# peteroh23/ModulationDetectionCNN

Measured on AMD Instinct MI355X. Metric: I/Q frames/sec (2x128, VT-CNN2, batch=2^20), higher is better.
Workload: dtype bf16; 1 GPU; vtcnn2-c11-bf16-n2^20; topology=vtcnn2, classes=11, frames_per_gpu=1048576, global_batch=1048576, parallelism=batch-shard x1 (no collective), outputs=softmax probabilities f32 + argmax int32, frames_per_forward_call=1048576, full=False

## Files before the change

modulationdetectioncnn_amd/csrc/vtcnn2_bf16_sched.hip:

```cpp
#include "vtcnn2_bf16_common.h"
#include "vtcnn2_sched_common.h"

#include <cmath>
#include <cstdlib>
#include <type_traits>

namespace mdc {

namespace {

constexpr int kNV = 24;

struct SchedState {
    u32x4 Wv[kNV];
    u32x4 Wa[kWFrags - kNV];
    f32x4 bias[5];
    u32x4 A1[2];
    unsigned Bf[2][2][2][4];
    f32x16 X[2];
    f32x4 rp[4];
    float rc[4];
    float tprev;
    u32x4 L0[3];
    u32x4 L1;
    unsigned cb[4];
    unsigned wr_addr, rd_addr, rc_addr, im_addr;
    int gs;
};

template <int SP, int J, int I, bool PAD = false>
__device__ __forceinline__ void sch_tap(SchedState& st, f32x4 (&acc)[5]) {
    constexpr int CT = 1 - I / 10, BB = (I / 5) % 2, OT = I % 5;
    constexpr int IDX = ((CT * 3 + J) * 2 + BB) * 5 + OT;
    const u32x4 b = u32x4{st.Bf[SP][CT][BB][0], st.Bf[SP][CT][BB][1], st.Bf[SP][CT][BB][2], st.Bf[SP][CT][BB][3]};
    if constexpr (J == 0 && I < 5) {
        if constexpr (IDX < kNV) asm volatile("v_mfma_f32_16x16x32_bf16 %0, %1, %2, %3" : "=&a"(acc[OT]) : "v"(st.Wv[IDX]), "v"(b), "a"(st.bias[OT]));
        else asm volatile("v_mfma_f32_16x16x32_bf16 %0, %1, %2, %3" : "=&a"(acc[OT]) : "a"(st.Wa[IDX - kNV]), "v"(b), "a"(st.bias[OT]));
    } else if constexpr (PAD) {
        static_assert(IDX >= kNV, "padded form written for the AGPR-resident fragments only");
        asm volatile("s_nop 1\n\tv_mfma_f32_16x16x32_bf16 %0, %1, %2, %0" : "+a"(acc[OT]) : "a"(st.Wa[IDX - kNV]), "v"(b));
    } else {
        if constexpr (IDX < kNV) asm volatile("v_mfma_f32_16x16x32_bf16 %0, %1, %2, %0" : "+a"(acc[OT]) : "v"(st.Wv[IDX]), "v"(b));
        else asm volatile("v_mfma_f32_16x16x32_bf16 %0, %1, %2, %0" : "+a"(acc[OT]) : "a"(st.Wa[IDX - kNV]), "v"(b));
    }
}
template <int SP, int U>
__device__ __forceinline__ void sch_packop(SchedState& st) {
    constexpr int CT = U >> 3, j = U & 7;
    unsigned& d = st.Bf[SP][CT][j >> 2][j & 3];
    const float lo = st.X[CT][2 * j], hi = st.X[CT][2 * j + 1];
    asm volatile("v_cvt_pk_bf16_f32 %0, %1, %2 clamp" : "=v"(d) : "v"(lo), "v"(hi));
}
template <int V12, bool FIRST, bool LAST, int ABL, bool RANGE = false>
__device__ __forceinline__ void sch_step(SchedState& st, int v, int q, unsigned short* fbase, f32x4 (&acc)[3][5], int wlo = 0) {
    constexpr int PAR = V12 & 1, PN = 1 - PAR;
    constexpr int R1 = (V12 + 1) & 3, S0 = ((V12 + 1) >> 2) % 3, SN = (S0 + 1) % 3;
    constexpr bool kLoadEven = (V12 & 3) == 1 && !LAST, kLoadOdd = (V12 & 3) == 3 && !LAST;
    constexpr int LSLOT = ((V12 >> 2) + 1) % 3;
    constexpr bool kExch = ABL != 2 && ABL != 6, kFin = ABL != 3 && ABL != 6, kC1 = ABL != 5 && ABL != 6;
    f32x4 (&a2)[5] = acc[V12 % 3];
    f32x4 (&a1)[5] = acc[(V12 + 1) % 3];
    f32x4 (&a0)[5] = acc[(V12 + 2) % 3];
    const unsigned load_addr = st.im_addr + ((v >> 2) * 16 + (kLoadEven ? 16 : 24));
    FinTmp ft;
    FinOut fo;
    constexpr int OP = (V12 + 1) & 1;
#define FIN(K) do { if (!FIRST && kFin) sch_fin_clamp<K, OP>(st, ft, fo); } while (0)
#define PREP(I) do { if (!LAST && kC1 && ABL != 11) sch_prep<R1, S0, SN, I>(st); } while (0)
#define C1M(CT) do { if (!LAST && kC1) sch_conv1_mfma<R1, S0, CT>(st); } while (0)
#define ST(W) do { if (!FIRST && kFin && (W == 0 || OP == 1)) { if (ABL == 7) { if (W == 0) asm volatile("" ::"v"(fo.o0), "v"(fo.o1)); else asm volatile("" ::"v"(fo.tt)); } else if (!RANGE || v - 1 >= wlo) sch_store<W>(fo, fbase, v - 1, q, st.gs); } } while (0)
#define WR(OT) do { if (kExch && ABL != 8) sch_part_write<PAR, OT>(st, a2[OT]); } while (0)
#define PK(N) do { if (!LAST && kC1 && ABL != 10) sch_packop<PN, N>(st); } while (0)
#define RD(R) do { if (kExch && ABL != 9) sch_red_load1<PAR, R>(st); } while (0)
#define LD() do { if (kC1 && ABL != 11) { if (kLoadEven) sch_load_even<LSLOT>(st, load_addr); else if (kLoadOdd) sch_load_odd(st, load_addr); } } while (0)
#ifdef MDC_F8_PROBE_HALF_BARRIER
    constexpr bool kHalfBarrierSkip = (V12 & 1) == 1;
#else
    constexpr bool kHalfBarrierSkip = false;
#endif
#define HANDOFF() do { \
        if (ABL == 1 || kHalfBarrierSkip) asm volatile("s_waitcnt lgkmcnt(0)" ::: "memory"); \
        else if (kExch) asm volatile("s_waitcnt lgkmcnt(0)\n\ts_barrier" ::: "memory"); \
        asm volatile("" ::"a"(a2[0]), "a"(a2[1]), "a"(a2[2]), "a"(a2[3]), "a"(a2[4])); } while (0)
    sch_wait_lds(st);
    sch_tap<PAR, 2, 0, RANGE && (V12 == 1 || V12 == 2)>(st, a2); FIN(0);
    sch_tap<PAR, 2, 1>(st, a2); FIN(1);
    sch_tap<PAR, 2, 2>(st, a2); FIN(2);
    sch_tap<PAR, 2, 3>(st, a2); FIN(3);
    sch_tap<PAR, 2, 4>(st, a2); FIN(4);
    sch_tap<PAR, 2, 5>(st, a2); FIN(5);
    sch_tap<PAR, 2, 6>(st, a2); FIN(6);
    sch_tap<PAR, 2, 7>(st, a2); FIN(7);
    sch_tap<PAR, 2, 8>(st, a2); FIN(8);
    sch_tap<PAR, 2, 9>(st, a2); FIN(9);
    sch_tap<PAR, 2, 10>(st, a2); FIN(10);
    sch_tap<PAR, 2, 11>(st, a2); FIN(11);
    sch_tap<PAR, 2, 12>(st, a2); FIN(12);
    sch_tap<PAR, 2, 13>(st, a2); FIN(13);
    sch_tap<PAR, 2, 14>(st, a2); FIN(14);
    sch_tap<PAR, 2, 15>(st, a2); FIN(15);
    sch_tap<PAR, 2, 16>(st, a2); PREP(0);
    sch_tap<PAR, 2, 17>(st, a2); PREP(1);
    sch_tap<PAR, 2, 18>(st, a2); PREP(2);
    sch_tap<PAR, 2, 19>(st, a2); PREP(3);
    C1M(0); WR(0); FIN(16); FIN(17);
    C1M(1); WR(1);
    sch_tap<PAR, 1, 0>(st, a1); ST(0);
    sch_tap<PAR, 1, 1>(st, a1); WR(2);
    sch_tap<PAR, 1, 2>(st, a1); ST(1);
    sch_tap<PAR, 1, 3>(st, a1); PK(0);
    sch_tap<PAR, 1, 4>(st, a1); WR(3);
    sch_tap<PAR, 1, 5>(st, a1); PK(1);
    sch_tap<PAR, 1, 6>(st, a1); PK(2);
    sch_tap<PAR, 1, 7>(st, a1); WR(4);
    sch_tap<PAR, 1, 8>(st, a1); PK(3);
    sch_tap<PAR, 1, 9>(st, a1); PK(4);
    sch_tap<PAR, 1, 10>(st, a1); PK(5);
    sch_tap<PAR, 1, 11>(st, a1); PK(6);
    sch_tap<PAR, 1, 12>(st, a1); PK(7);
    sch_tap<PAR, 1, 13>(st, a1); PK(8);
    sch_tap<PAR, 1, 14>(st, a1); PK(9);
    sch_tap<PAR, 1, 15>(st, a1); PK(10);
    sch_tap<PAR, 1, 16>(st, a1); PK(11);
    sch_tap<PAR, 1, 17>(st, a1); PK(12);
    sch_tap<PAR, 1, 18>(st, a1); PK(13);
    sch_tap<PAR, 1, 19>(st, a1); PK(14);
    sch_tap<PAR, 0, 0>(st, a0); PK(15);
    sch_tap<PAR, 0, 1>(st, a0);
    sch_tap<PAR, 0, 2>(st, a0);
    sch_tap<PAR, 0, 3>(st, a0);
    sch_tap<PAR, 0, 4>(st, a0);
    sch_tap<PAR, 0, 5>(st, a0);
    sch_tap<PAR, 0, 6>(st, a0); HANDOFF();
    sch_tap<PAR, 0, 7>(st, a0); RD(0);
    sch_tap<PAR, 0, 8>(st, a0); RD(1);
    sch_tap<PAR, 0, 9>(st, a0); RD(2);
    sch_tap<PAR, 0, 10>(st, a0); RD(3);
    sch_tap<PAR, 0, 11>(st, a0); RD(4);
    sch_tap<PAR, 0, 12>(st, a0); RD(5);
    sch_tap<PAR, 0, 13>(st, a0); RD(6);
    sch_tap<PAR, 0, 14>(st, a0); RD(7);
    sch_tap<PAR, 0, 15>(st, a0); LD();
    sch_tap<PAR, 0, 16>(st, a0);
    sch_tap<PAR, 0, 17>(st, a0);
    sch_tap<PAR, 0, 18>(st, a0);
    sch_tap<PAR, 0, 19>(st, a0);
    if (ABL == 10 && !LAST) asm volatile("" ::"v"(st.X[0]), "v"(st.X[1]));
#undef FIN
#undef PREP
#undef C1M
#undef ST
#undef WR
#undef PK
#undef RD
#undef LD
#undef HANDOFF
}

template <int ABL, bool U8 = false, bool RANGE = false>
__global__ __launch_bounds__(256, 1) void vt_conv_bf16_sched_kernel(const float* __restrict__ x, long n,
                                                                    const u32x4* __restrict__ wq, const u32x4* __restrict__ a1q,
                                                                    const float* __restrict__ b2, unsigned short* __restrict__ feat,
                                                                    long hop2 = 256, float scale = 0.f) {
    extern __shared__ __attribute__((aligned(16))) unsigned char smem[];
    unsigned* img = reinterpret_cast<unsigned*>(smem);
    const int tid = threadIdx.x, lane = tid & 63;
    const int q = __builtin_amdgcn_readfirstlane(tid >> 6);
    const int nl = lane & 15, g = lane >> 4;

    SchedState st;
#pragma unroll
    for (int i = 0; i < kWFrags; ++i) {
        const u32x4 w = wq[(q * kWFrags + i) * 64 + lane];
        if (i < kNV) { st.Wv[i] = w; asm volatile("" : "+v"(st.Wv[i])); }
        else { st.Wa[i - kNV] = w; asm volatile("" : "+a"(st.Wa[i - kNV])); }
    }
    st.A1[0] = a1q[(q * 2 + 0) * 64 + lane];
    st.A1[1] = a1q[(q * 2 + 1) * 64 + lane];
#pragma unroll
    for (int ot = 0; ot < 5; ++ot) {
        const f32x4 b = *reinterpret_cast<const f32x4*>(b2 + 16 * ot + 4 * g);
        st.bias[ot] = q == 0 ? b : f32x4{0.f, 0.f, 0.f, 0.f};
        asm volatile("" : "+a"(st.bias[ot]));
    }
    const unsigned part_lds = (unsigned)(size_t)(__attribute__((address_space(3))) unsigned char*)(smem + (size_t)2 * kSImgWords * 4);
    const unsigned img_lds = (unsigned)(size_t)(__attribute__((address_space(3))) unsigned char*)smem;
    auto entry = [](int f, int gg) { return 8 * (4 * (f >> 3) + gg) + ((f & 7) ^ (gg >> 1)); };
    const int fs = lane >> 2, gs = lane & 3;
    st.gs = gs;
    st.wr_addr = part_lds + (q * 5 * 64 + entry(nl, g)) * 16;
    st.rd_addr = part_lds + (q * 64 + entry(fs, gs)) * 16;
    st.rc_addr = part_lds + (4 * 64 + entry(fs, q)) * 16 + gs * 4;
#pragma unroll
    for (int k = 0; k < 4; ++k) { st.rp[k] = f32x4{0.f, 0.f, 0.f, 0.f}; st.rc[k] = 0.f; }
#pragma unroll
    for (int s = 0; s < 3; ++s) st.L0[s] = u32x4{0u, 0u, 0u, 0u};
    st.L1 = u32x4{0u, 0u, 0u, 0u};
    st.cb[0] = st.cb[1] = st.cb[2] = st.cb[3] = 0u;
    st.tprev = 0.f;

    for (int i = tid; i < 2 * kSImgWords; i += 256) img[i] = ((((i / kS) & 63) >= 32) && ((i % kS) & 1)) ? 0x3F803F80u : 0u;
    __syncthreads();
    const long ngroups = (n + 15) >> 4;
    long grp = blockIdx.x;
    if (grp < ngroups)
        for (int k = 0; k < 4; ++k) sch_stage_write(k, stage_decode<U8>(stage_load<U8>(k, x, n, grp * 16, tid, hop2), tid, scale), n, grp * 16, img, tid);
    __syncthreads();
    const int rng = RANGE ? (int)blockIdx.y : 0;
    const int S = 12 * rng;
    const int wlo = rng ? S + 2 : 0;

    int buf = 0;
    for (; grp < ngroups; grp += gridDim.x, buf ^= 1) {
        st.im_addr = img_lds + (buf * kSImgWords + lane * kS) * 4;
        unsigned short* fbase = feat + (grp * 16 + fs) * (long)(kW2 * kC2);
        const long gnext = RANGE ? ngroups : grp + gridDim.x;
        f32x4 acc[3][5];
        {
            const u32x4 zero = u32x4{0u, 0u, 0u, 0u};
#pragma unroll
            for (int b = 0; b < 5; ++b) {
                asm volatile("s_nop 1\n\tv_mfma_f32_16x16x32_bf16 %0, %1, %1, %2" : "=&a"(acc[0][b]) : "v"(zero), "a"(st.bias[b]));
                asm volatile("v_mfma_f32_16x16x32_bf16 %0, %1, %1, %2" : "=&a"(acc[1][b]) : "v"(zero), "a"(st.bias[b]));
            }
        }

        sch_load_even<0>(st, st.im_addr + (S >> 2) * 16);
        sch_load_odd(st, st.im_addr + (S >> 2) * 16 + 8);
        sch_wait_lds(st);
        sch_conv1_mfma<0, 0, 0>(st); sch_conv1_mfma<0, 0, 1>(st);
        asm volatile("s_nop 7\n\ts_nop 7\n\ts_nop 7\n\ts_nop 7\n\ts_nop 7\n\ts_nop 7\n\ts_nop 7\n\ts_nop 7" : "+v"(st.X[0]), "+v"(st.X[1]));
        [&]<int... N>(std::integer_sequence<int, N...>) { (sch_packop<0, N>(st), ...); }(std::make_integer_sequence<int, 16>{});
        asm volatile("s_nop 1");

        sch_step<0, true, false, ABL, RANGE>(st, S, q, fbase, acc, wlo);
        const int iters = RANGE ? (rng < 10 ? 1 : 0) : 10;
        int v = S + 1;
        typename StageRaw<U8>::type sv{};
        for (int it = 0; it < iters; ++it, v += 12) {
            if constexpr (!RANGE) {
                if (it >= 6 && gnext < ngroups) sch_stage_write(it - 6, stage_decode<U8>(sv, tid, scale), n, gnext * 16, img + (buf ^ 1) * kSImgWords, tid);
                if (it >= 5 && it < 9 && gnext < ngroups) sv = stage_load<U8>(it - 5, x, n, gnext * 16, tid, hop2);
            }
            sch_step<1, false, false, ABL, RANGE>(st, v + 0, q, fbase, acc, wlo);
            sch_step<2, false, false, ABL, RANGE>(st, v + 1, q, fbase, acc, wlo);
            sch_step<3, false, false, ABL, RANGE>(st, v + 2, q, fbase, acc, wlo);
            sch_step<4, false, false, ABL, RANGE>(st, v + 3, q, fbase, acc, wlo);
            sch_step<5, false, false, ABL, RANGE>(st, v + 4, q, fbase, acc, wlo);
            sch_step<6, false, false, ABL, RANGE>(st, v + 5, q, fbase, acc, wlo);
            sch_step<7, false, false, ABL, RANGE>(st, v + 6, q, fbase, acc, wlo);
            sch_step<8, false, false, ABL, RANGE>(st, v + 7, q, fbase, acc, wlo);
            sch_step<9, false, false, ABL, RANGE>(st, v + 8, q, fbase, acc, wlo);
            sch_step<10, false, false, ABL, RANGE>(st, v + 9, q, fbase, acc, wlo);
            sch_step<11, false, false, ABL, RANGE>(st, v + 10, q, fbase, acc, wlo);
            sch_step<0, false, false, ABL, RANGE>(st, v + 11, q, fbase, acc, wlo);
        }
        const int vt = RANGE ? v : 121;
        sch_step<1, false, false, ABL, RANGE>(st, vt, q, fbase, acc, wlo);
        if constexpr (RANGE) {
            if (rng < 10) {
                FinOut fo;
                sch_wait_lds(st);
                sch_fin_all_clamp<1>(st, fo);
                sch_store<0>(fo, fbase, vt, q, st.gs);
                sch_store<1>(fo, fbase, vt, q, st.gs);
                asm volatile("s_nop 7\n\ts_nop 7" ::"a"(acc[0][0]), "a"(acc[1][0]), "a"(acc[2][0]));
                __syncthreads();
                continue;
            }
        }
        sch_step<2, false, false, ABL, RANGE>(st, 122, q, fbase, acc, wlo);
        sch_step<3, false, false, ABL, RANGE>(st, 123, q, fbase, acc, wlo);
        sch_step<4, false, false, ABL, RANGE>(st, 124, q, fbase, acc, wlo);
        sch_step<5, false, false, ABL, RANGE>(st, 125, q, fbase, acc, wlo);
        sch_step<6, false, false, ABL, RANGE>(st, 126, q, fbase, acc, wlo);
        sch_step<7, false, false, ABL, RANGE>(st, 127, q, fbase, acc, wlo);
        sch_step<8, false, false, ABL, RANGE>(st, 128, q, fbase, acc, wlo);
        sch_step<9, false, true, ABL, RANGE>(st, 129, q, fbase, acc, wlo);
        auto finish_store = [&](auto odd, int w) {
            FinOut fo;
            sch_wait_lds(st);
            sch_fin_all_clamp<decltype(odd)::value>(st, fo);
            sch_store<0>(fo, fbase, w, q, st.gs);
            if constexpr (decltype(odd)::value) sch_store<1>(fo, fbase, w, q, st.gs);
        };
        using Even = std::integral_constant<int, 0>;
        using Odd = std::integral_constant<int, 1>;
        finish_store(Odd{}, 129);
        asm volatile("s_nop 7\n\ts_nop 7");
        sch_part_write<0, 0>(st, acc[1][0]); sch_part_write<0, 1>(st, acc[1][1]); sch_part_write<0, 2>(st, acc[1][2]);
        sch_part_write<0, 3>(st, acc[1][3]); sch_part_write<0, 4>(st, acc[1][4]);
        asm volatile("s_waitcnt lgkmcnt(0)\n\ts_barrier" ::: "memory");
        sch_red_load<0>(st);
        asm volatile("" ::"a"(acc[1][0]), "a"(acc[1][1]), "a"(acc[1][2]), "a"(acc[1][3]), "a"(acc[1][4]));
        finish_store(Even{}, 130);
        sch_part_write<1, 0>(st, acc[2][0]); sch_part_write<1, 1>(st, acc[2][1]); sch_part_write<1, 2>(st, acc[2][2]);
        sch_part_write<1, 3>(st, acc[2][3]); sch_part_write<1, 4>(st, acc[2][4]);
        asm volatile("s_waitcnt lgkmcnt(0)\n\ts_barrier" ::: "memory");
        sch_red_load<1>(st);
        asm volatile("" ::"a"(acc[2][0]), "a"(acc[2][1]), "a"(acc[2][2]), "a"(acc[2][3]), "a"(acc[2][4]));
        finish_store(Odd{}, 131);
        __syncthreads();
    }
}

}

int vtcnn2_bf16_pack_sched(mdc_model* m) {
    const float* k1 = m->hk[0].data();
    const float* b1 = m->hb[0].data();
    const float* k2 = m->hk[1].data();
    int rc;
    std::vector<unsigned short> wq((size_t)4 * kWFrags * 64 * 8);
    for (int q = 0; q < 4; ++q)
        for (int ct = 0; ct < 2; ++ct)
            for (int j = 0; j < 3; ++j)
                for (int bb = 0; bb < 2; ++bb)
                    for (int ot = 0; ot < 5; ++ot)
                        for (int lane = 0; lane < 64; ++lane)
                            for (int jj = 0; jj < 8; ++jj) {
                                const int o = 16 * ot + (lane & 15), kg = lane >> 4, h = kg & 1, r = 8 * bb + jj;
                                const int ch = 64 * q + 32 * ct + 8 * (r >> 2) + 4 * (kg >> 1) + (r & 3);
                                const size_t idx = ((((size_t)q * kWFrags + ((ct * 3 + j) * 2 + bb) * 5 + ot) * 64) + lane) * 8 + jj;
                                wq[idx] = f2bf(k2[(((size_t)o * kC1 + ch) * 2 + h) * 3 + j]);
                            }
    if ((rc = upload(m, 6, wq.data(), wq.size() * 2))) return rc;
    std::vector<unsigned short> a1((size_t)4 * 2 * 64 * 8, 0);
    for (int q = 0; q < 4; ++q)
        for (int ct = 0; ct < 2; ++ct)
            for (int lane = 0; lane < 64; ++lane) {
                const int ch = 64 * q + 32 * ct + (lane & 31), khalf = lane >> 5;
                unsigned short* d = &a1[(((size_t)q * 2 + ct) * 64 + lane) * 8];
                const float sc = std::ldexp(1.f, -kFeatShift);
                unsigned short th[3], tl[3];
                for (int t = 0; t < 3; ++t) {
                    th[t] = f2bf(k1[ch * 3 + t] * sc);
                    tl[t] = f2bf(k1[ch * 3 + t] * sc - bf2f(th[t]));
                }
                if (khalf == 0) {
                    d[0] = th[0]; d[1] = th[1]; d[2] = th[0]; d[3] = th[1]; d[4] = th[2]; d[6] = th[2];
                } else {
                    const unsigned short bh = f2bf(b1[ch] * sc);
                    d[0] = tl[0]; d[1] = tl[1]; d[2] = bh; d[3] = f2bf(b1[ch] * sc - bf2f(bh)); d[4] = tl[2];
                }
            }
    return upload(m, 7, a1.data(), a1.size() * 2);
}

int vtcnn2_bf16_conv_sched(const mdc_model* m, const float* x, int64_t n, void* feat, hipStream_t s, long hop2, float scale) {
    const long ngroups = (n + 15) / 16;
    const unsigned grid = (unsigned)(ngroups < 256 ? ngroups : 256);
#define MDC_LAUNCH_SCHED_V(U, R, GRID) do { \
    MDC_HIP(hipFuncSetAttribute(reinterpret_cast<const void*>(vt_conv_bf16_sched_kernel<0, U, R>), hipFuncAttributeMaxDynamicSharedMemorySize, (int)kSchedLds)); \
    hipLaunchKernelGGL((vt_conv_bf16_sched_kernel<0, U, R>), GRID, dim3(256), kSchedLds, s, x, (long)n, \
                       static_cast<const u32x4*>(m->d_pack[6]), static_cast<const u32x4*>(m->d_pack[7]), \
                       static_cast<const float*>(m->d_pack[2]), static_cast<unsigned short*>(feat), hop2 > 0 ? hop2 : 256L, scale); \
    MDC_HIP(hipGetLastError()); return MDC_OK; } while (0)
    if (n <= kConvRangeFrames) {
        if (hop2 > 0) MDC_LAUNCH_SCHED_V(true, true, dim3((unsigned)ngroups, 11));
        else MDC_LAUNCH_SCHED_V(false, true, dim3((unsigned)ngroups, 11));
    }
    if (hop2 > 0) MDC_LAUNCH_SCHED_V(true, false, dim3(grid));
#undef MDC_LAUNCH_SCHED_V
#define MDC_LAUNCH_SCHED(A) do { \
    MDC_HIP(hipFuncSetAttribute(reinterpret_cast<const void*>(vt_conv_bf16_sched_kernel<A>), hipFuncAttributeMaxDynamicSharedMemorySize, (int)kSchedLds)); \
    hipLaunchKernelGGL(vt_conv_bf16_sched_kernel<A>, dim3(grid), dim3(256), kSchedLds, s, x, (long)n, \
                       static_cast<const u32x4*>(m->d_pack[6]), static_cast<const u32x4*>(m->d_pack[7]), \
                       static_cast<const float*>(m->d_pack[2]), static_cast<unsigned short*>(feat), 256L, 0.f); } while (0)
#ifdef MDC_ABLATIONS
    static const int abl = getenv("MDC_ABLATE_S") ? atoi(getenv("MDC_ABLATE_S")) : 0;
    switch (abl) { case 1: MDC_LAUNCH_SCHED(1); break; case 2: MDC_LAUNCH_SCHED(2); break; case 3: MDC_LAUNCH_SCHED(3); break;
                   case 5: MDC_LAUNCH_SCHED(5); break; case 6: MDC_LAUNCH_SCHED(6); break; case 7: MDC_LAUNCH_SCHED(7); break;
                   case 8: MDC_LAUNCH_SCHED(8); break; case 9: MDC_LAUNCH_SCHED(9); break; case 10: MDC_LAUNCH_SCHED(10); break;
                   case 11: MDC_LAUNCH_SCHED(11); break; default: MDC_LAUNCH_SCHED(0); }
#else
    MDC_LAUNCH_SCHED(0);
#endif
#undef MDC_LAUNCH_SCHED
    MDC_HIP(hipGetLastError());
    return MDC_OK;
}

}
```

modulationdetectioncnn_amd/csrc/vtcnn2_sched_common.h:

```cpp
#pragma once
#include "vtcnn2_bf16_common.h"

#include <type_traits>
#include <utility>

namespace mdc {

namespace {

constexpr int kS = 140;
constexpr int kSImgWords = 64 * kS;
constexpr long kConvRangeFrames = 1024;
constexpr size_t kSchedLds = (size_t)2 * kSImgWords * 4 + (size_t)2 * kPartFloats * 4;

using f32x16 = __attribute__((ext_vector_type(16))) float;

template <int SLOT, class S>
__device__ __forceinline__ void sch_load_even(S& st, unsigned entry_addr) {
    asm volatile("ds_read_b128 %0, %1" : "=v"(st.L0[SLOT]) : "v"(entry_addr) : "memory");
}
template <class S>
__device__ __forceinline__ void sch_load_odd(S& st, unsigned entry_addr) {
    asm volatile("ds_read2_b64 %0, %1 offset0:0 offset1:1" : "=v"(st.L1) : "v"(entry_addr) : "memory");
}
template <int R, int S0, int SN, int I, class S>
__device__ __forceinline__ void sch_prep(S& st) {
    if constexpr (R == 1 || R == 3) {
        const unsigned w0 = R == 1 ? st.L0[S0][0] : st.L1[0], w1 = R == 1 ? st.L0[S0][1] : st.L1[1];
        const unsigned w2 = R == 1 ? st.L0[S0][2] : st.L1[2], w3 = R == 1 ? st.L0[S0][3] : st.L1[3];
        const unsigned w4 = R == 1 ? st.L1[2] : st.L0[SN][2], w5 = R == 1 ? st.L1[3] : st.L0[SN][3];
        unsigned& d = st.cb[I];
        if constexpr (I == 0) asm volatile("v_alignbit_b32 %0, %1, %2, 16" : "=v"(d) : "v"(w2), "v"(w0));
        else if constexpr (I == 1) asm volatile("v_alignbit_b32 %0, %1, %2, 16" : "=v"(d) : "v"(w3), "v"(w1));
        else if constexpr (I == 2) asm volatile("v_alignbit_b32 %0, %1, %2, 16" : "=v"(d) : "v"(w4), "v"(w2));
        else asm volatile("v_alignbit_b32 %0, %1, %2, 16" : "=v"(d) : "v"(w5), "v"(w3));
    }
}
template <int R, int S0, int CT, class S>
__device__ __forceinline__ void sch_conv1_mfma(S& st) {
    const u32x4 b = R == 0 ? st.L0[S0] : R == 2 ? st.L1 : u32x4{st.cb[0], st.cb[1], st.cb[2], st.cb[3]};
    asm volatile("v_mfma_f32_32x32x16_bf16 %0, %1, %2, 0" : "=&v"(st.X[CT]) : "v"(st.A1[CT]), "v"(b));
}
template <int PB, int OT, class S>
__device__ __forceinline__ void sch_part_write(S& st, const f32x4& a) {
    asm volatile("ds_write_b128 %0, %1 offset:%2" ::"v"(st.wr_addr), "a"(a), "i"(PB * kPartFloats * 4 + OT * 1024) : "memory");
}
template <int PB, int R, class S>
__device__ __forceinline__ void sch_red_load1(S& st) {
    constexpr int K = R >> 1;
    if constexpr ((R & 1) == 0) asm volatile("ds_read_b128 %0, %1 offset:%2" : "=v"(st.rp[K]) : "v"(st.rd_addr), "i"(PB * kPartFloats * 4 + K * 5120) : "memory");
    else asm volatile("ds_read_b32 %0, %1 offset:%2" : "=v"(st.rc[K]) : "v"(st.rc_addr), "i"(PB * kPartFloats * 4 + K * 5120) : "memory");
}
template <int PB, class S>
__device__ __forceinline__ void sch_red_load(S& st) {
    sch_red_load1<PB, 0>(st); sch_red_load1<PB, 1>(st); sch_red_load1<PB, 2>(st); sch_red_load1<PB, 3>(st);
    sch_red_load1<PB, 4>(st); sch_red_load1<PB, 5>(st); sch_red_load1<PB, 6>(st); sch_red_load1<PB, 7>(st);
}
template <class S>
__device__ __forceinline__ void sch_wait_lds(S& st) {
    asm volatile("s_waitcnt lgkmcnt(0)"
                 : "+v"(st.rp[0]), "+v"(st.rp[1]), "+v"(st.rp[2]), "+v"(st.rp[3]), "+v"(st.rc[0]), "+v"(st.rc[1]), "+v"(st.rc[2]),
                   "+v"(st.rc[3]), "+v"(st.L0[0]), "+v"(st.L0[1]), "+v"(st.L0[2]), "+v"(st.L1)
                 :: "memory");
}
struct FinOut { unsigned o0, o1, tt; };
struct FinTmp { float s[4], u[4], a, b, t; };
constexpr int kFeatShift = 32;

template <int K, int ODD, class S>
__device__ __forceinline__ void sch_fin_clamp(S& st, FinTmp& f, FinOut& out) {
    if constexpr (K < 4) asm volatile("v_add_f32 %0, %1, %2" : "=v"(f.s[K]) : "v"(st.rp[0][K]), "v"(st.rp[1][K]));
    else if constexpr (K < 8) asm volatile("v_add_f32 %0, %1, %2" : "=v"(f.u[K - 4]) : "v"(st.rp[2][K - 4]), "v"(st.rp[3][K - 4]));
    else if constexpr (K < 12) asm volatile("v_add_f32 %0, %0, %1" : "+v"(f.s[K - 8]) : "v"(f.u[K - 8]));
    else if constexpr (K == 12) asm volatile("v_cvt_pk_bf16_f32 %0, %1, %2 clamp" : "=v"(out.o0) : "v"(f.s[0]), "v"(f.s[1]));
    else if constexpr (K == 13) asm volatile("v_cvt_pk_bf16_f32 %0, %1, %2 clamp" : "=v"(out.o1) : "v"(f.s[2]), "v"(f.s[3]));
    else if constexpr (K == 14) asm volatile("v_add_f32 %0, %1, %2" : "=v"(f.a) : "v"(st.rc[0]), "v"(st.rc[1]));
    else if constexpr (K == 15) asm volatile("v_add_f32 %0, %1, %2" : "=v"(f.b) : "v"(st.rc[2]), "v"(st.rc[3]));
    else if constexpr (K == 16) {
        if constexpr (ODD) asm volatile("v_add_f32 %0, %1, %2" : "=v"(f.t) : "v"(f.a), "v"(f.b));
        else asm volatile("v_add_f32 %0, %1, %2" : "=v"(st.tprev) : "v"(f.a), "v"(f.b));
    } else if constexpr (ODD) asm volatile("v_cvt_pk_bf16_f32 %0, %1, %2 clamp" : "=v"(out.tt) : "v"(st.tprev), "v"(f.t));
}
template <int ODD, class S>
__device__ __forceinline__ void sch_fin_all_clamp(S& st, FinOut& out) {
    FinTmp f;
    [&]<int... K>(std::integer_sequence<int, K...>) { (sch_fin_clamp<K, ODD>(st, f, out), ...); }(std::make_integer_sequence<int, 18>{});
}

template <int WHICH>
__device__ __forceinline__ void sch_store(const FinOut& fo, unsigned short* frow, int w, int q, int gs) {
    unsigned short* pair = frow + (long)(w >> 1) * (2 * kC2);
    if constexpr (WHICH == 0) *reinterpret_cast<u32x2*>(pair + (w & 1) * 64 + 16 * q + 4 * gs) = u32x2{fo.o0, fo.o1};
    else *reinterpret_cast<unsigned*>(pair + 128 + 2 * (4 * q + gs)) = fo.tt;
}

__device__ __forceinline__ void sch_stage_write(int k, float4 v, long n, long frame0, unsigned* __restrict__ im, int tid) {
    const int idx = tid + 256 * k;
    const int i = idx >> 6, l = idx & 63;
    if (frame0 + i >= n) v = make_float4(0.f, 0.f, 0.f, 0.f);
    const int h = l >> 5, m = l & 31;
    const float xs[4] = {v.x, v.y, v.z, v.w};
#pragma unroll
    for (int e = 0; e < 2; ++e) {
        const float a = xs[2 * e], b = xs[2 * e + 1];
        const unsigned hi = pack2(a, b);
        const float ah = __uint_as_float(hi << 16), bh = __uint_as_float(hi & 0xFFFF0000u);
        const unsigned lo = pack2(a - ah, b - bh);
        unsigned* d = im + (i + 16 * h) * kS + 2 * (2 * m + 1 + e);
        *reinterpret_cast<u32x2*>(d) = u32x2{hi, lo};
        d[32 * kS] = hi;
    }
}


}

}
```

Measured before the change: 40.18 million frames/s.

## Interleave next-group input staging into MFMA slots and overlap group seams

Next-group frame staging (global load, bf16 hi/lo split, LDS write) is now done with inline asm scattered into spare slots between MFMA taps over the last four 12-step blocks, replacing the separate bulk stage_load/stage_write passes. The group-seam prologue is restructured: the first step folds bias into its MFMAs instead of issuing zero-MFMA bias inits, and the next group's initial image load is issued at the end of the previous group's epilogue, with one barrier wait reordered. The aim is to hide staging and seam latency behind matrix work, at the cost of more live registers and fragile hand-tuned waitcnt counts. New ablation modes 12-15 are added and the half-barrier probe is removed.

New measurement: 40.42 million frames/s (median of 6 runs). No clear change (+0.6%).

```diff
diff --git a/modulationdetectioncnn_amd/csrc/vtcnn2_bf16_sched.hip b/modulationdetectioncnn_amd/csrc/vtcnn2_bf16_sched.hip
--- a/modulationdetectioncnn_amd/csrc/vtcnn2_bf16_sched.hip
+++ b/modulationdetectioncnn_amd/csrc/vtcnn2_bf16_sched.hip
@@ -26,14 +26,31 @@
     unsigned cb[4];
     unsigned wr_addr, rd_addr, rc_addr, im_addr;
     int gs;
+    f32x4 sx;
+    float xm[4];
+    unsigned th[4], shi[2], slo[2];
+    unsigned sg_off, stw_lo, stw_hi;
+    const float* sg_frame;
+    unsigned sg_mask;
 };
 
-template <int SP, int J, int I, bool PAD = false>
+template <int V12, int G, int NST>
+__device__ __forceinline__ void sch_stg_slot(SchedState& st) {
+    if constexpr (V12 == 1 && G == 1) sch_stg_load(st, st.sg_frame);
+    else if constexpr (V12 == 6 && G == 1) sch_stg_wait<NST>(st);
+    else if constexpr (V12 == 6 && G >= 2 && G <= 5) sch_stg_valu<G - 2>(st, st.sg_mask);
+    else if constexpr (V12 == 6 && G >= 16) sch_stg_valu<G - 12>(st, st.sg_mask);
+    else if constexpr (V12 == 7 && G <= 5) sch_stg_valu<G + 7>(st, st.sg_mask);
+    else if constexpr (V12 == 7 && G >= 16 && G <= 18) sch_stg_valu<G - 3>(st, st.sg_mask);
+    else if constexpr (V12 >= 8 && V12 <= 10 && G == 1) sch_stg_write<V12 - 8>(st);
+}
+
+template <int SP, int J, int I, bool PAD = false, bool BIAS = (J == 0 && I < 5)>
 __device__ __forceinline__ void sch_tap(SchedState& st, f32x4 (&acc)[5]) {
     constexpr int CT = 1 - I / 10, BB = (I / 5) % 2, OT = I % 5;
     constexpr int IDX = ((CT * 3 + J) * 2 + BB) * 5 + OT;
     const u32x4 b = u32x4{st.Bf[SP][CT][BB][0], st.Bf[SP][CT][BB][1], st.Bf[SP][CT][BB][2], st.Bf[SP][CT][BB][3]};
-    if constexpr (J == 0 && I < 5) {
+    if constexpr (BIAS) {
         if constexpr (IDX < kNV) asm volatile("v_mfma_f32_16x16x32_bf16 %0, %1, %2, %3" : "=&a"(acc[OT]) : "v"(st.Wv[IDX]), "v"(b), "a"(st.bias[OT]));
         else asm volatile("v_mfma_f32_16x16x32_bf16 %0, %1, %2, %3" : "=&a"(acc[OT]) : "a"(st.Wa[IDX - kNV]), "v"(b), "a"(st.bias[OT]));
     } else if constexpr (PAD) {
@@ -51,7 +68,7 @@
     const float lo = st.X[CT][2 * j], hi = st.X[CT][2 * j + 1];
     asm volatile("v_cvt_pk_bf16_f32 %0, %1, %2 clamp" : "=v"(d) : "v"(lo), "v"(hi));
 }
-template <int V12, bool FIRST, bool LAST, int ABL, bool RANGE = false>
+template <int V12, bool FIRST, bool LAST, int ABL, bool RANGE = false, bool STG = false>
 __device__ __forceinline__ void sch_step(SchedState& st, int v, int q, unsigned short* fbase, f32x4 (&acc)[3][5], int wlo = 0) {
     constexpr int PAR = V12 & 1, PN = 1 - PAR;
     constexpr int R1 = (V12 + 1) & 3, S0 = ((V12 + 1) >> 2) % 3, SN = (S0 + 1) % 3;
@@ -72,22 +89,19 @@
 #define WR(OT) do { if (kExch && ABL != 8) sch_part_write<PAR, OT>(st, a2[OT]); } while (0)
 #define PK(N) do { if (!LAST && kC1 && ABL != 10) sch_packop<PN, N>(st); } while (0)
 #define RD(R) do { if (kExch && ABL != 9) sch_red_load1<PAR, R>(st); } while (0)
+    constexpr int kStoresBehindLoad = kFin && ABL != 7 ? 8 : 0;
+#define SG(G) do { if constexpr (STG) sch_stg_slot<V12, G, kStoresBehindLoad>(st); } while (0)
 #define LD() do { if (kC1 && ABL != 11) { if (kLoadEven) sch_load_even<LSLOT>(st, load_addr); else if (kLoadOdd) sch_load_odd(st, load_addr); } } while (0)
-#ifdef MDC_F8_PROBE_HALF_BARRIER
-    constexpr bool kHalfBarrierSkip = (V12 & 1) == 1;
-#else
-    constexpr bool kHalfBarrierSkip = false;
-#endif
 #define HANDOFF() do { \
-        if (ABL == 1 || kHalfBarrierSkip) asm volatile("s_waitcnt lgkmcnt(0)" ::: "memory"); \
+        if (ABL == 1) asm volatile("s_waitcnt lgkmcnt(0)" ::: "memory"); \
         else if (kExch) asm volatile("s_waitcnt lgkmcnt(0)\n\ts_barrier" ::: "memory"); \
         asm volatile("" ::"a"(a2[0]), "a"(a2[1]), "a"(a2[2]), "a"(a2[3]), "a"(a2[4])); } while (0)
     sch_wait_lds(st);
-    sch_tap<PAR, 2, 0, RANGE && (V12 == 1 || V12 == 2)>(st, a2); FIN(0);
-    sch_tap<PAR, 2, 1>(st, a2); FIN(1);
-    sch_tap<PAR, 2, 2>(st, a2); FIN(2);
-    sch_tap<PAR, 2, 3>(st, a2); FIN(3);
-    sch_tap<PAR, 2, 4>(st, a2); FIN(4);
+    sch_tap<PAR, 2, 0, RANGE && (V12 == 1 || V12 == 2), FIRST>(st, a2); FIN(0);
+    sch_tap<PAR, 2, 1, false, FIRST>(st, a2); FIN(1);
+    sch_tap<PAR, 2, 2, false, FIRST>(st, a2); FIN(2);
+    sch_tap<PAR, 2, 3, false, FIRST>(st, a2); FIN(3);
+    sch_tap<PAR, 2, 4, false, FIRST>(st, a2); FIN(4);
     sch_tap<PAR, 2, 5>(st, a2); FIN(5);
     sch_tap<PAR, 2, 6>(st, a2); FIN(6);
     sch_tap<PAR, 2, 7>(st, a2); FIN(7);
@@ -105,11 +119,11 @@
     sch_tap<PAR, 2, 19>(st, a2); PREP(3);
     C1M(0); WR(0); FIN(16); FIN(17);
     C1M(1); WR(1);
-    sch_tap<PAR, 1, 0>(st, a1); ST(0);
-    sch_tap<PAR, 1, 1>(st, a1); WR(2);
-    sch_tap<PAR, 1, 2>(st, a1); ST(1);
-    sch_tap<PAR, 1, 3>(st, a1); PK(0);
-    sch_tap<PAR, 1, 4>(st, a1); WR(3);
+    sch_tap<PAR, 1, 0, false, FIRST>(st, a1); ST(0);
+    sch_tap<PAR, 1, 1, false, FIRST>(st, a1); WR(2);
+    sch_tap<PAR, 1, 2, false, FIRST>(st, a1); ST(1);
+    sch_tap<PAR, 1, 3, false, FIRST>(st, a1); PK(0);
+    sch_tap<PAR, 1, 4, false, FIRST>(st, a1); WR(3);
     sch_tap<PAR, 1, 5>(st, a1); PK(1);
     sch_tap<PAR, 1, 6>(st, a1); PK(2);
     sch_tap<PAR, 1, 7>(st, a1); WR(4);
@@ -126,11 +140,11 @@
     sch_tap<PAR, 1, 18>(st, a1); PK(13);
     sch_tap<PAR, 1, 19>(st, a1); PK(14);
     sch_tap<PAR, 0, 0>(st, a0); PK(15);
-    sch_tap<PAR, 0, 1>(st, a0);
-    sch_tap<PAR, 0, 2>(st, a0);
-    sch_tap<PAR, 0, 3>(st, a0);
-    sch_tap<PAR, 0, 4>(st, a0);
-    sch_tap<PAR, 0, 5>(st, a0);
+    sch_tap<PAR, 0, 1>(st, a0); SG(1);
+    sch_tap<PAR, 0, 2>(st, a0); SG(2);
+    sch_tap<PAR, 0, 3>(st, a0); SG(3);
+    sch_tap<PAR, 0, 4>(st, a0); SG(4);
+    sch_tap<PAR, 0, 5>(st, a0); SG(5);
     sch_tap<PAR, 0, 6>(st, a0); HANDOFF();
     sch_tap<PAR, 0, 7>(st, a0); RD(0);
     sch_tap<PAR, 0, 8>(st, a0); RD(1);
@@ -141,10 +155,10 @@
     sch_tap<PAR, 0, 13>(st, a0); RD(6);
     sch_tap<PAR, 0, 14>(st, a0); RD(7);
     sch_tap<PAR, 0, 15>(st, a0); LD();
-    sch_tap<PAR, 0, 16>(st, a0);
-    sch_tap<PAR, 0, 17>(st, a0);
-    sch_tap<PAR, 0, 18>(st, a0);
-    sch_tap<PAR, 0, 19>(st, a0);
+    sch_tap<PAR, 0, 16>(st, a0); SG(16);
+    sch_tap<PAR, 0, 17>(st, a0); SG(17);
+    sch_tap<PAR, 0, 18>(st, a0); SG(18);
+    sch_tap<PAR, 0, 19>(st, a0); SG(19);
     if (ABL == 10 && !LAST) asm volatile("" ::"v"(st.X[0]), "v"(st.X[1]));
 #undef FIN
 #undef PREP
@@ -154,6 +168,7 @@
 #undef PK
 #undef RD
 #undef LD
+#undef SG
 #undef HANDOFF
 }
 
@@ -210,50 +225,71 @@
     const int S = 12 * rng;
     const int wlo = rng ? S + 2 : 0;
 
+    constexpr bool kStage = ABL != 12 && ABL != 14, kSeam = ABL != 13 && ABL != 14;
+    constexpr bool kGapStage = !U8 && !RANGE && kStage && ABL != 15;
+    st.sg_off = lane * 16;
+    const unsigned stg_lane = img_lds + (16 * (lane >> 5) * kS + 4 * (lane & 31) + 2) * 4;
     int buf = 0;
+    if constexpr (!RANGE && kSeam) { sch_load_even<0>(st, img_lds + lane * kS * 4); sch_load_odd(st, img_lds + lane * kS * 4 + 8); }
     for (; grp < ngroups; grp += gridDim.x, buf ^= 1) {
-        st.im_addr = img_lds + (buf * kSImgWords + lane * kS) * 4;
+        st.im_addr = img_lds + ((kStage ? buf : 0) * kSImgWords + lane * kS) * 4;
         unsigned short* fbase = feat + (grp * 16 + fs) * (long)(kW2 * kC2);
         const long gnext = RANGE ? ngroups : grp + gridDim.x;
         f32x4 acc[3][5];
-        {
-            const u32x4 zero = u32x4{0u, 0u, 0u, 0u};
-#pragma unroll
-            for (int b = 0; b < 5; ++b) {
-                asm volatile("s_nop 1\n\tv_mfma_f32_16x16x32_bf16 %0, %1, %1, %2" : "=&a"(acc[0][b]) : "v"(zero), "a"(st.bias[b]));
-                asm volatile("v_mfma_f32_16x16x32_bf16 %0, %1, %1, %2" : "=&a"(acc[1][b]) : "v"(zero), "a"(st.bias[b]));
+
+        if constexpr (kSeam) {
+            if constexpr (RANGE) {
+                sch_load_even<0>(st, st.im_addr + (S >> 2) * 16);
+                sch_load_odd(st, st.im_addr + (S >> 2) * 16 + 8);
             }
+            sch_wait_lds(st);
+            sch_conv1_mfma<0, 0, 0>(st); sch_conv1_mfma<0, 0, 1>(st);
+            asm volatile("s_nop 7\n\ts_nop 7\n\ts_nop 7\n\ts_nop 7\n\ts_nop 7\n\ts_nop 7\n\ts_nop 7\n\ts_nop 7" : "+v"(st.X[0]), "+v"(st.X[1]));
+            [&]<int... N>(std::integer_sequence<int, N...>) { (sch_packop<0, N>(st), ...); }(std::make_integer_sequence<int, 16>{});
+            asm volatile("s_nop 1");
+        } else {
+            for (int i = 0; i < 16; ++i) asm volatile("" : "=v"(st.Bf[0][i >> 3][(i >> 2) & 1][i & 3]));
         }
-
-        sch_load_even<0>(st, st.im_addr + (S >> 2) * 16);
-        sch_load_odd(st, st.im_addr + (S >> 2) * 16 + 8);
-        sch_wait_lds(st);
-        sch_conv1_mfma<0, 0, 0>(st); sch_conv1_mfma<0, 0, 1>(st);
-        asm volatile("s_nop 7\n\ts_nop 7\n\ts_nop 7\n\ts_nop 7\n\ts_nop 7\n\ts_nop 7\n\ts_nop 7\n\ts_nop 7" : "+v"(st.X[0]), "+v"(st.X[1]));
-        [&]<int... N>(std::integer_sequence<int, N...>) { (sch_packop<0, N>(st), ...); }(std::make_integer_sequence<int, 16>{});
-        asm volatile("s_nop 1");
 
         sch_step<0, true, false, ABL, RANGE>(st, S, q, fbase, acc, wlo);
         const int iters = RANGE ? (rng < 10 ? 1 : 0) : 10;
         int v = S + 1;
-        typename StageRaw<U8>::type sv{};
-        for (int it = 0; it < iters; ++it, v += 12) {
-            if constexpr (!RANGE) {
-                if (it >= 6 && gnext < ngroups) sch_stage_write(it - 6, stage_decode<U8>(sv, tid, scale), n, gnext * 16, img + (buf ^ 1) * kSImgWords, tid);
-                if (it >= 5 && it < 9 && gnext < ngroups) sv = stage_load<U8>(it - 5, x, n, gnext * 16, tid, hop2);
+        auto body12 = [&](auto stg) {
+            constexpr bool G = decltype(stg)::value;
+            sch_step<1, false, false, ABL, RANGE, G>(st, v + 0, q, fbase, acc, wlo);
+            sch_step<2, false, false, ABL, RANGE, G>(st, v + 1, q, fbase, acc, wlo);
+            sch_step<3, false, false, ABL, RANGE, G>(st, v + 2, q, fbase, acc, wlo);
+            sch_step<4, false, false, ABL, RANGE, G>(st, v + 3, q, fbase, acc, wlo);
+            sch_step<5, false, false, ABL, RANGE, G>(st, v + 4, q, fbase, acc, wlo);
+            sch_step<6, false, false, ABL, RANGE, G>(st, v + 5, q, fbase, acc, wlo);
+            sch_step<7, false, false, ABL, RANGE, G>(st, v + 6, q, fbase, acc, wlo);
+            sch_step<8, false, false, ABL, RANGE, G>(st, v + 7, q, fbase, acc, wlo);
+            sch_step<9, false, false, ABL, RANGE, G>(st, v + 8, q, fbase, acc, wlo);
+            sch_step<10, false, false, ABL, RANGE, G>(st, v + 9, q, fbase, acc, wlo);
+            sch_step<11, false, false, ABL, RANGE, G>(st, v + 10, q, fbase, acc, wlo);
+            sch_step<0, false, false, ABL, RANGE, G>(st, v + 11, q, fbase, acc, wlo);
+        };
+        if constexpr (kGapStage) {
+            const bool has_next = gnext < ngroups;
+            for (int it = has_next ? 4 : 0; it < 10; ++it, v += 12) body12(std::false_type{});
+            if (has_next)
+                for (int k = 0; k < 4; ++k, v += 12) {
+                    const long f = gnext * 16 + q + 4 * k;
+                    st.sg_frame = x + (f < n ? f : n - 1) * kFrameFloats;
+                    st.sg_mask = f < n ? ~0u : 0u;
+                    st.stw_lo = stg_lane + ((buf ^ 1) * kSImgWords + (q + 4 * k) * kS) * 4;
+                    st.stw_hi = st.stw_lo + 32 * kS * 4;
+                    body12(std::true_type{});
+                }
+        } else {
+            typename StageRaw<U8>::type sv{};
+            for (int it = 0; it < iters; ++it, v += 12) {
+                if constexpr (!RANGE && kStage) {
+                    if (it >= 6 && gnext < ngroups) sch_stage_write(it - 6, stage_decode<U8>(sv, tid, scale), n, gnext * 16, img + (buf ^ 1) * kSImgWords, tid);
+                    if (it >= 5 && it < 9 && gnext < ngroups) sv = stage_load<U8>(it - 5, x, n, gnext * 16, tid, hop2);
+                }
+                body12(std::false_type{});
             }
-            sch_step<1, false, false, ABL, RANGE>(st, v + 0, q, fbase, acc, wlo);
-            sch_step<2, false, false, ABL, RANGE>(st, v + 1, q, fbase, acc, wlo);
-            sch_step<3, false, false, ABL, RANGE>(st, v + 2, q, fbase, acc, wlo);
-            sch_step<4, false, false, ABL, RANGE>(st, v + 3, q, fbase, acc, wlo);
-            sch_step<5, false, false, ABL, RANGE>(st, v + 4, q, fbase, acc, wlo);
-            sch_step<6, false, false, ABL, RANGE>(st, v + 5, q, fbase, acc, wlo);
-            sch_step<7, false, false, ABL, RANGE>(st, v + 6, q, fbase, acc, wlo);
-            sch_step<8, false, false, ABL, RANGE>(st, v + 7, q, fbase, acc, wlo);
-            sch_step<9, false, false, ABL, RANGE>(st, v + 8, q, fbase, acc, wlo);
-            sch_step<10, false, false, ABL, RANGE>(st, v + 9, q, fbase, acc, wlo);
-            sch_step<11, false, false, ABL, RANGE>(st, v + 10, q, fbase, acc, wlo);
-            sch_step<0, false, false, ABL, RANGE>(st, v + 11, q, fbase, acc, wlo);
         }
         const int vt = RANGE ? v : 121;
         sch_step<1, false, false, ABL, RANGE>(st, vt, q, fbase, acc, wlo);
@@ -288,17 +324,28 @@
         using Odd = std::integral_constant<int, 1>;
         finish_store(Odd{}, 129);
         asm volatile("s_nop 7\n\ts_nop 7");
+        if constexpr (!kSeam) {
+            asm volatile("" ::"a"(acc[1][0]), "a"(acc[1][1]), "a"(acc[1][2]), "a"(acc[1][3]), "a"(acc[1][4]));
+            asm volatile("" ::"a"(acc[2][0]), "a"(acc[2][1]), "a"(acc[2][2]), "a"(acc[2][3]), "a"(acc[2][4]));
+            __syncthreads();
+            continue;
+        }
         sch_part_write<0, 0>(st, acc[1][0]); sch_part_write<0, 1>(st, acc[1][1]); sch_part_write<0, 2>(st, acc[1][2]);
         sch_part_write<0, 3>(st, acc[1][3]); sch_part_write<0, 4>(st, acc[1][4]);
         asm volatile("s_waitcnt lgkmcnt(0)\n\ts_barrier" ::: "memory");
         sch_red_load<0>(st);
         asm volatile("" ::"a"(acc[1][0]), "a"(acc[1][1]), "a"(acc[1][2]), "a"(acc[1][3]), "a"(acc[1][4]));
-        finish_store(Even{}, 130);
         sch_part_write<1, 0>(st, acc[2][0]); sch_part_write<1, 1>(st, acc[2][1]); sch_part_write<1, 2>(st, acc[2][2]);
         sch_part_write<1, 3>(st, acc[2][3]); sch_part_write<1, 4>(st, acc[2][4]);
-        asm volatile("s_waitcnt lgkmcnt(0)\n\ts_barrier" ::: "memory");
+        finish_store(Even{}, 130);
+        asm volatile("s_barrier" ::: "memory");
+        asm volatile("" ::"a"(acc[2][0]), "a"(acc[2][1]), "a"(acc[2][2]), "a"(acc[2][3]), "a"(acc[2][4]));
         sch_red_load<1>(st);
-        asm volatile("" ::"a"(acc[2][0]), "a"(acc[2][1]), "a"(acc[2][2]), "a"(acc[2][3]), "a"(acc[2][4]));
+        if constexpr (!RANGE) {
+            const unsigned im_next = img_lds + ((kStage ? buf ^ 1 : 0) * kSImgWords + lane * kS) * 4;
+            sch_load_even<0>(st, im_next);
+            sch_load_odd(st, im_next + 8);
+        }
         finish_store(Odd{}, 131);
         __syncthreads();
     }
@@ -372,7 +419,8 @@
     switch (abl) { case 1: MDC_LAUNCH_SCHED(1); break; case 2: MDC_LAUNCH_SCHED(2); break; case 3: MDC_LAUNCH_SCHED(3); break;
                    case 5: MDC_LAUNCH_SCHED(5); break; case 6: MDC_LAUNCH_SCHED(6); break; case 7: MDC_LAUNCH_SCHED(7); break;
                    case 8: MDC_LAUNCH_SCHED(8); break; case 9: MDC_LAUNCH_SCHED(9); break; case 10: MDC_LAUNCH_SCHED(10); break;
-                   case 11: MDC_LAUNCH_SCHED(11); break; default: MDC_LAUNCH_SCHED(0); }
+                   case 11: MDC_LAUNCH_SCHED(11); break; case 12: MDC_LAUNCH_SCHED(12); break; case 13: MDC_LAUNCH_SCHED(13); break;
+                   case 14: MDC_LAUNCH_SCHED(14); break; case 15: MDC_LAUNCH_SCHED(15); break; default: MDC_LAUNCH_SCHED(0); }
 #else
     MDC_LAUNCH_SCHED(0);
 #endif
diff --git a/modulationdetectioncnn_amd/csrc/vtcnn2_sched_common.h b/modulationdetectioncnn_amd/csrc/vtcnn2_sched_common.h
--- a/modulationdetectioncnn_amd/csrc/vtcnn2_sched_common.h
+++ b/modulationdetectioncnn_amd/csrc/vtcnn2_sched_common.h
@@ -112,6 +112,31 @@
     }
 }
 
+template <class S>
+__device__ __forceinline__ void sch_stg_load(S& st, const float* frame) {
+    asm volatile("global_load_dwordx4 %0, %1, %2" : "=v"(st.sx) : "v"(st.sg_off), "s"(frame) : "memory");
+}
+template <int N, class S>
+__device__ __forceinline__ void sch_stg_wait(S& st) {
+    asm volatile("s_waitcnt vmcnt(%1)" : "+v"(st.sx) : "n"(N) : "memory");
+}
+template <int K, class S>
+__device__ __forceinline__ void sch_stg_valu(S& st, unsigned mask) {
+    constexpr int e = K & 1;
+    if constexpr (K < 4) asm volatile("v_and_b32 %0, %1, %2" : "=v"(st.xm[K]) : "v"(mask), "v"(st.sx[K]));
+    else if constexpr (K < 6) asm volatile("v_cvt_pk_bf16_f32 %0, %1, %2" : "=v"(st.shi[e]) : "v"(st.xm[2 * e]), "v"(st.xm[2 * e + 1]));
+    else if constexpr (K < 8) asm volatile("v_lshlrev_b32 %0, 16, %1" : "=v"(st.th[2 * e]) : "v"(st.shi[e]));
+    else if constexpr (K < 10) asm volatile("v_and_b32 %0, 0xffff0000, %1" : "=v"(st.th[2 * e + 1]) : "v"(st.shi[e]));
+    else if constexpr (K < 14) asm volatile("v_sub_f32 %0, %0, %1" : "+v"(st.xm[K - 10]) : "v"(st.th[K - 10]));
+    else asm volatile("v_cvt_pk_bf16_f32 %0, %1, %2" : "=v"(st.slo[e]) : "v"(st.xm[2 * e]), "v"(st.xm[2 * e + 1]));
+}
+template <int W, class S>
+__device__ __forceinline__ void sch_stg_write(S& st) {
+    if constexpr (W == 0) asm volatile("ds_write2_b32 %0, %1, %2 offset1:1" ::"v"(st.stw_lo), "v"(st.shi[0]), "v"(st.slo[0]) : "memory");
+    else if constexpr (W == 1) asm volatile("ds_write2_b32 %0, %1, %2 offset0:2 offset1:3" ::"v"(st.stw_lo), "v"(st.shi[1]), "v"(st.slo[1]) : "memory");
+    else asm volatile("ds_write2_b32 %0, %1, %2 offset1:2" ::"v"(st.stw_hi), "v"(st.shi[0]), "v"(st.shi[1]) : "memory");
+}
+
 
 }
 
```
